# ZcsrenlongZ/Deblur4DGS

Hardware: AMD Instinct MI355X
Metric: Gaussians/s fwd+bwd, 288x512, N_exposure=8 (higher is better)
Workload: dtype f32; 1 GPU; cfg2: 300000 Gaussians (300000 dynamic), 6 motion bases, 512x288, N_exposure=8, 3+depth channels, fwd+bwd to all leaves; gaussians=300000, exposure_subsamples=8, parallelism=1 GPU, lazy_sort=off (auto), pre_roll_steps=30

## Files before the change

### deblur4dgs_amd/csrc/common.h

```cpp
#pragma once
#include <hip/hip_runtime.h>
#include <stdint.h>

#include "../../include/d4gs.h"

#define D4GS_WAVE 64
#define D4GS_MAX_K 32
#define D4GS_PROJ_BLOCK 256


#define D4GS_SSIM_WINDOW                                                                                                   \
  {0.00102838008447911, 0.007598758135239185, 0.03600077212843083, 0.10936068950970002, 0.2130055377112537, 0.26601172486179436, \
   0.2130055377112537,  0.10936068950970002,  0.03600077212843083, 0.007598758135239185, 0.00102838008447911}

void d4gs_set_error(const char *fmt, ...);
int d4gs_check_launch(const char *what);


__device__ __forceinline__ void mat3_mul(const float *A, const float *B, float *C) {
#pragma unroll
  for (int i = 0; i < 3; i++)
#pragma unroll
    for (int j = 0; j < 3; j++) C[i * 3 + j] = A[i * 3] * B[j] + A[i * 3 + 1] * B[3 + j] + A[i * 3 + 2] * B[6 + j];
}
__device__ __forceinline__ void mat3_mul_bt(const float *A, const float *B, float *C) {
#pragma unroll
  for (int i = 0; i < 3; i++)
#pragma unroll
    for (int j = 0; j < 3; j++)
      C[i * 3 + j] = A[i * 3] * B[j * 3] + A[i * 3 + 1] * B[j * 3 + 1] + A[i * 3 + 2] * B[j * 3 + 2];
}
__device__ __forceinline__ void mat3_mul_at(const float *A, const float *B, float *C) {
#pragma unroll
  for (int i = 0; i < 3; i++)
#pragma unroll
    for (int j = 0; j < 3; j++) C[i * 3 + j] = A[i] * B[j] + A[3 + i] * B[3 + j] + A[6 + i] * B[6 + j];
}

__device__ __forceinline__ void quat_to_rotmat(float w, float x, float y, float z, float *R) {
  R[0] = 1.f - 2.f * (y * y + z * z);
  R[1] = 2.f * (x * y - w * z);
  R[2] = 2.f * (x * z + w * y);
  R[3] = 2.f * (x * y + w * z);
  R[4] = 1.f - 2.f * (x * x + z * z);
  R[5] = 2.f * (y * z - w * x);
  R[6] = 2.f * (x * z - w * y);
  R[7] = 2.f * (y * z + w * x);
  R[8] = 1.f - 2.f * (x * x + y * y);
}

struct GS6 {
  float x[3], y[3], z[3];
  float inv_na, inv_nb;
  float d;
};
__device__ __forceinline__ void gram_schmidt(const float *r6, GS6 &o) {
  float na = sqrtf(r6[0] * r6[0] + r6[1] * r6[1] + r6[2] * r6[2]);
  o.inv_na = 1.f / fmaxf(na, 1e-12f);
#pragma unroll
  for (int i = 0; i < 3; i++) o.x[i] = r6[i] * o.inv_na;
  o.d = r6[3] * o.x[0] + r6[4] * o.x[1] + r6[5] * o.x[2];
  float bp[3];
#pragma unroll
  for (int i = 0; i < 3; i++) bp[i] = r6[3 + i] - o.d * o.x[i];
  float nb = sqrtf(bp[0] * bp[0] + bp[1] * bp[1] + bp[2] * bp[2]);
  o.inv_nb = 1.f / fmaxf(nb, 1e-12f);
#pragma unroll
  for (int i = 0; i < 3; i++) o.y[i] = bp[i] * o.inv_nb;
  o.z[0] = o.x[1] * o.y[2] - o.x[2] * o.y[1];
  o.z[1] = o.x[2] * o.y[0] - o.x[0] * o.y[2];
  o.z[2] = o.x[0] * o.y[1] - o.x[1] * o.y[0];
}

__device__ __forceinline__ int rq_choice(const float *R) {
  const float tr = R[0] + R[4] + R[8];
  int ch = 0;
  float best = R[0];
  if (R[4] > best) best = R[4], ch = 1;
  if (R[8] > best) best = R[8], ch = 2;
  if (tr > best) ch = 3;
  return ch;
}
template <int I>
__device__ __forceinline__ void rq_cand(const float *R, float *c) {
  const float tr = R[0] + R[4] + R[8];
  if constexpr (I == 3) {
    c[0] = R[7] - R[5], c[1] = R[2] - R[6], c[2] = R[3] - R[1], c[3] = 1.f + tr;
  } else {
    constexpr int J = (I + 1) % 3, Kk = (I + 2) % 3;
    c[I] = 1.f - tr + 2.f * R[I * 3 + I];
    c[J] = R[J * 3 + I] + R[I * 3 + J];
    c[Kk] = R[Kk * 3 + I] + R[I * 3 + Kk];
    c[3] = R[Kk * 3 + J] - R[J * 3 + Kk];
  }
}
template <int I>
__device__ __forceinline__ void rq_cand_adj(const float *vc, float *vR) {
  if constexpr (I == 3) {
    vR[7] += vc[0], vR[5] -= vc[0], vR[2] += vc[1], vR[6] -= vc[1], vR[3] += vc[2], vR[1] -= vc[2];
    vR[0] += vc[3], vR[4] += vc[3], vR[8] += vc[3];
  } else {
    constexpr int J = (I + 1) % 3, Kk = (I + 2) % 3;
    vR[I * 3 + I] += vc[I], vR[J * 3 + J] -= vc[I], vR[Kk * 3 + Kk] -= vc[I];
    vR[J * 3 + I] += vc[J], vR[I * 3 + J] += vc[J];
    vR[Kk * 3 + I] += vc[Kk], vR[I * 3 + Kk] += vc[Kk];
    vR[Kk * 3 + J] += vc[3], vR[J * 3 + Kk] -= vc[3];
  }
}
__device__ __forceinline__ void rq_cand_dyn(int ch, const float *R, float *c) {
  if (ch == 0) rq_cand<0>(R, c);
  else if (ch == 1) rq_cand<1>(R, c);
  else if (ch == 2) rq_cand<2>(R, c);
  else rq_cand<3>(R, c);
}
__device__ __forceinline__ void rq_cand_adj_dyn(int ch, const float *vc, float *vR) {
  if (ch == 0) rq_cand_adj<0>(vc, vR);
  else if (ch == 1) rq_cand_adj<1>(vc, vR);
  else if (ch == 2) rq_cand_adj<2>(vc, vR);
  else rq_cand_adj<3>(vc, vR);
}
__device__ __forceinline__ void quat_mul(const float *p, const float *q, float *r) {
  r[0] = p[0] * q[0] - p[1] * q[1] - p[2] * q[2] - p[3] * q[3];
  r[1] = p[0] * q[1] + p[1] * q[0] + p[2] * q[3] - p[3] * q[2];
  r[2] = p[0] * q[2] - p[1] * q[3] + p[2] * q[0] + p[3] * q[1];
  r[3] = p[0] * q[3] + p[1] * q[2] - p[2] * q[1] + p[3] * q[0];
}
__device__ __forceinline__ void quat_mul_adj(const float *p, const float *q, const float *vr, float *vp, float *vq) {
  vp[0] = vr[0] * q[0] + vr[1] * q[1] + vr[2] * q[2] + vr[3] * q[3];
  vp[1] = -vr[0] * q[1] + vr[1] * q[0] - vr[2] * q[3] + vr[3] * q[2];
  vp[2] = -vr[0] * q[2] + vr[1] * q[3] + vr[2] * q[0] - vr[3] * q[1];
  vp[3] = -vr[0] * q[3] - vr[1] * q[2] + vr[2] * q[1] + vr[3] * q[0];
  vq[0] = vr[0] * p[0] + vr[1] * p[1] + vr[2] * p[2] + vr[3] * p[3];
  vq[1] = -vr[0] * p[1] + vr[1] * p[0] + vr[2] * p[3] - vr[3] * p[2];
  vq[2] = -vr[0] * p[2] - vr[1] * p[3] + vr[2] * p[0] + vr[3] * p[1];
  vq[3] = -vr[0] * p[3] + vr[1] * p[2] - vr[2] * p[1] + vr[3] * p[0];
}
struct PoseQ {
  int ch;
  float p[4];
  float inv_nc;
  float out[4];
  float inv_nr;
};
__device__ __forceinline__ void pose_quat(const float *Rd, const float *qh, PoseQ &o) {
  float c[4];
  o.ch = rq_choice(Rd);
  rq_cand_dyn(o.ch, Rd, c);
  o.inv_nc = 1.f / sqrtf(c[0] * c[0] + c[1] * c[1] + c[2] * c[2] + c[3] * c[3]);
  o.p[0] = c[3] * o.inv_nc, o.p[1] = c[0] * o.inv_nc, o.p[2] = c[1] * o.inv_nc, o.p[3] = c[2] * o.inv_nc;
  float r[4];
  quat_mul(o.p, qh, r);
  o.inv_nr = 1.f / fmaxf(sqrtf(r[0] * r[0] + r[1] * r[1] + r[2] * r[2] + r[3] * r[3]), 1e-12f);
#pragma unroll
  for (int i = 0; i < 4; i++) o.out[i] = r[i] * o.inv_nr;
}
__device__ __forceinline__ void pose_quat_adj(const PoseQ &o, const float *qh, const float *v_out, float *vRd, float *v_qh) {
  const float dt = v_out[0] * o.out[0] + v_out[1] * o.out[1] + v_out[2] * o.out[2] + v_out[3] * o.out[3];
  float vr[4], vp[4], vq[4];
#pragma unroll
  for (int i = 0; i < 4; i++) vr[i] = (v_out[i] - dt * o.out[i]) * o.inv_nr;
  quat_mul_adj(o.p, qh, vr, vp, vq);
#pragma unroll
  for (int i = 0; i < 4; i++) v_qh[i] += vq[i];
  const float dp = vp[0] * o.p[0] + vp[1] * o.p[1] + vp[2] * o.p[2] + vp[3] * o.p[3];
  float vc[4];
  vc[0] = (vp[1] - dp * o.p[1]) * o.inv_nc, vc[1] = (vp[2] - dp * o.p[2]) * o.inv_nc;
  vc[2] = (vp[3] - dp * o.p[3]) * o.inv_nc, vc[3] = (vp[0] - dp * o.p[0]) * o.inv_nc;
  rq_cand_adj_dyn(o.ch, vc, vRd);
}

__device__ __forceinline__ void tile_rect(float mx, float my, int radius, int tw, int th, int &x0, int &y0, int &x1,
                                          int &y1) {
  const float inv = 1.0f / D4GS_TILE;
  float tx = mx * inv, ty = my * inv, tr = (float)radius * inv;
  x0 = (int)fminf(fmaxf(floorf(tx - tr), 0.f), (float)tw);
  y0 = (int)fminf(fmaxf(floorf(ty - tr), 0.f), (float)th);
  x1 = (int)fminf(fmaxf(ceilf(tx + tr), 0.f), (float)tw);
  y1 = (int)fminf(fmaxf(ceilf(ty + tr), 0.f), (float)th);
}

__device__ __forceinline__ void tight_rect(float mx, float my, float opac, float cov_xx, float cov_yy, int &x0, int &y0,
                                           int &x1, int &y1) {
  const float tau = __logf(255.f * opac) * 1.01f + 0.02f;
  if (!(tau > 0.f)) {
    x1 = x0, y1 = y0;
    return;
  }
  const float ex = sqrtf(2.f * tau * cov_xx) + 1e-3f, ey = sqrtf(2.f * tau * cov_yy) + 1e-3f;
  const float inv = 1.0f / D4GS_TILE;
  const float jx0 = ceilf(mx - ex - 0.5f), jx1 = floorf(mx + ex - 0.5f);
  const float jy0 = ceilf(my - ey - 0.5f), jy1 = floorf(my + ey - 0.5f);
  const int tx0 = (int)fmaxf(floorf(jx0 * inv), (float)x0), tx1 = (int)fminf(floorf(jx1 * inv) + 1.f, (float)x1);
  const int ty0 = (int)fmaxf(floorf(jy0 * inv), (float)y0), ty1 = (int)fminf(floorf(jy1 * inv) + 1.f, (float)y1);
  x0 = tx0, x1 = max(tx1, tx0), y0 = ty0, y1 = max(ty1, ty0);
  if (x1 == x0 || y1 == y0) x1 = x0, y1 = y0;
}

__device__ __forceinline__ bool d4gs_ellipse_hits_rect(float mx, float my, float a, float b, float c, float tau, float X0, float X1,
                                                       float Y0, float Y1) {
  const float U0 = X0 - mx, U1 = X1 - mx, V0 = Y0 - my, V1 = Y1 - my;
  const float uc = fminf(fmaxf(0.f, U0), U1), vc = fminf(fmaxf(0.f, V0), V1);
  if (uc == 0.f && vc == 0.f) return true;
  float best = 3.0e38f;
  if (uc != 0.f) {
    const float v = fminf(fmaxf(-b * uc * __builtin_amdgcn_rcpf(c), V0), V1);
    best = 0.5f * (a * uc * uc + c * v * v) + b * uc * v;
  }
  if (vc != 0.f) {
    const float u = fminf(fmaxf(-b * vc * __builtin_amdgcn_rcpf(a), U0), U1);
    best = fminf(best, 0.5f * (a * u * u + c * vc * vc) + b * u * vc);
  }
  return best <= tau * 1.001f + 1e-4f;
}

struct Cam {
  float R[9];
  float t[3];
  float fx, fy, cx, cy;
  float limx, limy;
};

__device__ __forceinline__ Cam load_cam(const float *V, const float *Km, int width, int height) {
  Cam c;
#pragma unroll
  for (int i = 0; i < 3; i++) {
#pragma unroll
    for (int j = 0; j < 3; j++) c.R[i * 3 + j] = V[i * 4 + j];
    c.t[i] = V[i * 4 + 3];
  }
  c.fx = Km[0], c.fy = Km[4], c.cx = Km[2], c.cy = Km[5];
  c.limx = 1.3f * (0.5f * (float)width / c.fx);
  c.limy = 1.3f * (0.5f * (float)height / c.fy);
  return c;
}

struct ProjOut {
  float pc[3];
  float M[9];
  float covc[6];
  float J02, J12;
  float rz;
  float a, b, c;
  float det;
  float det0;
  float mx, my;
  int radius;
  bool in_x, in_y;
};

__device__ __forceinline__ void project_instance(const Cam &cam, const float *mw, const float *Rm, const float *sc,
                                                 const D4gsDims &d, ProjOut &o) {
  o.radius = 0;
#pragma unroll
  for (int i = 0; i < 3; i++) o.pc[i] = cam.R[i * 3] * mw[0] + cam.R[i * 3 + 1] * mw[1] + cam.R[i * 3 + 2] * mw[2] + cam.t[i];
  float z = o.pc[2];
  if (!(z >= d.near_plane && z <= d.far_plane)) return;
  float W_[9];
  mat3_mul(cam.R, Rm, W_);
#pragma unroll
  for (int i = 0; i < 3; i++)
#pragma unroll
    for (int j = 0; j < 3; j++) o.M[i * 3 + j] = W_[i * 3 + j] * sc[j];
  const float *M = o.M;
  o.covc[0] = M[0] * M[0] + M[1] * M[1] + M[2] * M[2];
  o.covc[1] = M[0] * M[3] + M[1] * M[4] + M[2] * M[5];
  o.covc[2] = M[0] * M[6] + M[1] * M[7] + M[2] * M[8];
  o.covc[3] = M[3] * M[3] + M[4] * M[4] + M[5] * M[5];
  o.covc[4] = M[3] * M[6] + M[4] * M[7] + M[5] * M[8];
  o.covc[5] = M[6] * M[6] + M[7] * M[7] + M[8] * M[8];
  float rz = 1.f / z, rz2 = rz * rz;
  o.rz = rz;
  float xr = o.pc[0] * rz, yr = o.pc[1] * rz;
  o.in_x = (xr <= cam.limx) && (xr >= -cam.limx);
  o.in_y = (yr <= cam.limy) && (yr >= -cam.limy);
  float tx = z * fminf(cam.limx, fmaxf(-cam.limx, xr));
  float ty = z * fminf(cam.limy, fmaxf(-cam.limy, yr));
  float J00 = cam.fx * rz, J11 = cam.fy * rz;
  o.J02 = -cam.fx * tx * rz2;
  o.J12 = -cam.fy * ty * rz2;
  const float cxx = o.covc[0], cxy = o.covc[1], cxz = o.covc[2], cyy = o.covc[3], cyz = o.covc[4], czz = o.covc[5];
  float c00 = J00 * J00 * cxx + 2.f * J00 * o.J02 * cxz + o.J02 * o.J02 * czz;
  float c01 = J00 * J11 * cxy + J00 * o.J12 * cxz + o.J02 * J11 * cyz + o.J02 * o.J12 * czz;
  float c11 = J11 * J11 * cyy + 2.f * J11 * o.J12 * cyz + o.J12 * o.J12 * czz;
  o.a = c00 + d.eps2d;
  o.b = c01;
  o.c = c11 + d.eps2d;
  o.det = o.a * o.c - o.b * o.b;
  o.det0 = __builtin_fmaf(-c01, c01, c00 * c11);
  if (!(o.det > 0.f)) return;
  float mid = 0.5f * (o.a + o.c);
  float v1 = mid + sqrtf(fmaxf(0.01f, mid * mid - o.det));
  float radius = ceilf(3.f * sqrtf(v1));
  if (radius <= d.radius_clip) return;
  o.mx = cam.fx * o.pc[0] * rz + cam.cx;
  o.my = cam.fy * o.pc[1] * rz + cam.cy;
  if (o.mx + radius <= 0.f || o.mx - radius >= (float)d.width || o.my + radius <= 0.f ||
      o.my - radius >= (float)d.height)
    return;
  o.radius = (int)radius;
}

#ifndef D4GS_SEG_MAX
#define D4GS_SEG_MAX 8
#endif
#ifndef D4GS_SEG_UNIT
#define D4GS_SEG_UNIT 256
#endif
#ifndef D4GS_SEG_TILES_MAX
#define D4GS_SEG_TILES_MAX 1280
#endif
#ifndef D4GS_SEG_TILES_MAX_NARROW
#define D4GS_SEG_TILES_MAX_NARROW 5120
#endif
__host__ __device__ __forceinline__ int d4gs_seg_len(int len) {
  const int per = (len + D4GS_SEG_UNIT * D4GS_SEG_MAX - 1) / (D4GS_SEG_UNIT * D4GS_SEG_MAX);
  return D4GS_SEG_UNIT * (per > 1 ? per : 1);
}
int64_t d4gs_seg_state_elems(const D4gsDims *d);
bool d4gs_seg_on(const D4gsDims *d, const D4gsIsect *isect, const D4gsRaster *r);

struct LazyWs {
  int32_t *hist, *near, *pivot, *cur, *flag;
  uint32_t *zr;
  int nb;
};
__host__ __device__ __forceinline__ int d4gs_lazy_buckets(int tiles_per_subsample) { return tiles_per_subsample <= 2048 ? 8 : 4; }
__host__ __device__ __forceinline__ int64_t d4gs_lazy_ws_elems(int S, int tiles_per_subsample) {
  const int64_t T = (int64_t)S * tiles_per_subsample;
  return T * (d4gs_lazy_buckets(tiles_per_subsample) + 5) + 2 * (int64_t)S + 8;
}
__host__ __device__ __forceinline__ LazyWs d4gs_lazy_carve(int32_t *ws, int S, int tiles_per_subsample) {
  LazyWs w;
  const int64_t T = (int64_t)S * tiles_per_subsample;
  w.nb = d4gs_lazy_buckets(tiles_per_subsample);
  w.hist = ws, w.near = w.hist + T * w.nb, w.pivot = w.near + T, w.cur = w.pivot + T, w.flag = w.cur + 2 * T;
  w.zr = reinterpret_cast<uint32_t *>(w.flag + T);
  return w;
}
__device__ __forceinline__ int d4gs_depth_bucket(float depth, uint32_t zmin_bits, uint32_t zmax_bits, int nb) {
  const uint32_t b = __float_as_uint(depth);
  const uint64_t span = (uint64_t)(zmax_bits - zmin_bits) + 1u;
  const uint64_t off = b > zmin_bits ? (uint64_t)(b - zmin_bits) : 0u;
  const int k = (int)((off * (uint64_t)nb) / span);
  return k < nb ? k : nb - 1;
}

struct BlendAdj {
  const float *v_blended;
  const float *v_acc;
  const int8_t *win;
  uint64_t non_mean;
};
bool d4gs_lazy_on(const D4gsDims *d, const D4gsProjOut *out);
int d4gs_lazy_pivot_launch(const D4gsDims *d, const D4gsProjOut *out, int64_t near_target, hipStream_t stream);
int d4gs_lazy_far_sort(const D4gsDims *dims, const D4gsProjOut *proj, const D4gsIsect *isect, hipStream_t stream);
int d4gs_bases_table_launch(const D4gsDims *dims, const D4gsProjIn *in, float *btab, hipStream_t stream);
int d4gs_chunk_per_thread(const D4gsDims *d);
int d4gs_fused_scan_chunks(const D4gsDims *d);

struct ProfScope {
  int slot;
  hipStream_t stream;
  ProfScope(const char *name, hipStream_t s);
  ~ProfScope();
};

__device__ __forceinline__ float splat_sigma2(const float4 g1, float dx, float dy) {
#pragma clang fp contract(off)
  const float inner = __builtin_fmaf(g1.x, dx, g1.y * dy);
  return __builtin_fmaf(dx, inner, (g1.z * dy) * dy);
}
__device__ __forceinline__ float4 stage_conic(float a, float b, float c, float w) {
  constexpr float LOG2E_ = 1.4426950408889634f;
  return make_float4(a * (0.5f * LOG2E_), b * LOG2E_, c * (0.5f * LOG2E_), w);
}

#define D4GS_C1 "quad_perm:[1,0,3,2] row_mask:0xf bank_mask:0xf bound_ctrl:0"
#define D4GS_C2 "quad_perm:[2,3,0,1] row_mask:0xf bank_mask:0xf bound_ctrl:0"
#define D4GS_C3 "row_half_mirror row_mask:0xf bank_mask:0xf bound_ctrl:0"
#define D4GS_C4 "row_mirror row_mask:0xf bank_mask:0xf bound_ctrl:0"
#define D4GS_C5 "row_bcast:15 row_mask:0xa bank_mask:0xf"
#define D4GS_C6 "row_bcast:31 row_mask:0xc bank_mask:0xf"
#define D4GS_DA(i, c) "v_add_f32_dpp %" #i ", %" #i ", %" #i " " c "\n\t"
#define D4GS_S2(c) D4GS_DA(0, c) D4GS_DA(1, c) "s_nop 0\n\t"
#define D4GS_S1(c) D4GS_DA(0, c) "s_nop 1\n\t"

__device__ __forceinline__ float swap32_add(float a, float b) {
  auto r = __builtin_amdgcn_permlane32_swap(__float_as_uint(a), __float_as_uint(b), false, false);
  return __uint_as_float(r[0]) + __uint_as_float(r[1]);
}
__device__ __forceinline__ float swap16_add(float a, float b) {
  auto r = __builtin_amdgcn_permlane16_swap(__float_as_uint(a), __float_as_uint(b), false, false);
  return __uint_as_float(r[0]) + __uint_as_float(r[1]);
}
#define D4GS_R3(c) D4GS_DA(0, c) D4GS_DA(1, c) D4GS_DA(2, c)
__device__ __forceinline__ void rowsum3(float &a, float &b, float &c) {
  asm volatile("s_nop 1\n\t" D4GS_R3(D4GS_C1) D4GS_R3(D4GS_C2) D4GS_R3(D4GS_C3) D4GS_R3(D4GS_C4)
               : "+v"(a), "+v"(b), "+v"(c));
}
__device__ __forceinline__ void rowsum2(float &a, float &b) {
  asm volatile("s_nop 1\n\t" D4GS_S2(D4GS_C1) D4GS_S2(D4GS_C2) D4GS_S2(D4GS_C3) D4GS_S2(D4GS_C4) : "+v"(a), "+v"(b));
}
__device__ __forceinline__ void rowsum1(float &a) {
  asm volatile("s_nop 1\n\t" D4GS_S1(D4GS_C1) D4GS_S1(D4GS_C2) D4GS_S1(D4GS_C3) D4GS_S1(D4GS_C4) : "+v"(a));
}
__device__ __forceinline__ void bcast15(float &a) {
  asm volatile("s_nop 1\n\t" D4GS_DA(0, D4GS_C5) : "+v"(a));
}
__device__ __forceinline__ void bcast15_31(float &a) {
  asm volatile("s_nop 1\n\t" D4GS_DA(0, D4GS_C5) "s_nop 1\n\t" D4GS_DA(0, D4GS_C6) : "+v"(a));
}
template <int NR>
__device__ __forceinline__ void rowsum_all(float (&z)[NR]) {
  constexpr int n3 = NR / 3, r = NR % 3;
#pragma unroll
  for (int i = 0; i < n3; i++) rowsum3(z[3 * i], z[3 * i + 1], z[3 * i + 2]);
  if constexpr (r == 2) rowsum2(z[NR - 2], z[NR - 1]);
  if constexpr (r == 1) rowsum1(z[NR - 1]);
}
#ifndef D4GS_PACKED_LADDER
#define D4GS_PACKED_LADDER 1
#endif
#define D4GS_C7 "row_ror:4 row_mask:0xf bank_mask:0xf"
#define D4GS_C8 "row_ror:8 row_mask:0xf bank_mask:0xf"
#define D4GS_C5S "row_bcast:15 row_mask:0xa bank_mask:0x8"
#define D4GS_C6S "row_bcast:31 row_mask:0xc bank_mask:0x8"
template <bool SINGLE >
__device__ __forceinline__ float rowsum3_packed(float a, float b, float c) {
  const uint64_t odd = 0xaaaaaaaaaaaaaaaaull, l3 = 0x8888888888888888ull;
  if constexpr (SINGLE)
    asm volatile("s_nop 1\n\t" D4GS_R3(D4GS_C1) "v_cndmask_b32_e64 %0, %0, %1, %3\n\ts_nop 0\n\t" D4GS_DA(2, D4GS_C2) D4GS_DA(0, D4GS_C2)
                 "v_cndmask_b32_e64 %0, %0, %2, %4\n\ts_nop 1\n\t" D4GS_DA(0, D4GS_C7) "s_nop 1\n\t" D4GS_DA(0, D4GS_C8)
                 "s_nop 1\n\t" D4GS_DA(0, D4GS_C5S) "s_nop 1\n\t" D4GS_DA(0, D4GS_C6S)
                 : "+v"(a), "+v"(b), "+v"(c)
                 : "s"(odd), "s"(l3));
  else
    asm volatile("s_nop 1\n\t" D4GS_R3(D4GS_C1) "v_cndmask_b32_e64 %0, %0, %1, %3\n\ts_nop 0\n\t" D4GS_DA(2, D4GS_C2) D4GS_DA(0, D4GS_C2)
                 "v_cndmask_b32_e64 %0, %0, %2, %4\n\ts_nop 1\n\t" D4GS_DA(0, D4GS_C7) "s_nop 1\n\t" D4GS_DA(0, D4GS_C8)
                 "s_nop 1\n\t" D4GS_DA(0, D4GS_C5S)
                 : "+v"(a), "+v"(b), "+v"(c)
                 : "s"(odd), "s"(l3));
  return a;
}
template <bool PAIR>
__device__ __forceinline__ float rowsum2_packed(float a, float b) {
  const uint64_t odd = 0xaaaaaaaaaaaaaaaaull;
  if constexpr (PAIR)
    asm volatile("s_nop 1\n\t" D4GS_DA(0, D4GS_C1) D4GS_DA(1, D4GS_C1) "v_cndmask_b32_e64 %0, %0, %1, %2\n\ts_nop 1\n\t" D4GS_DA(0, D4GS_C2)
                 "s_nop 1\n\t" D4GS_DA(0, D4GS_C7) "s_nop 1\n\t" D4GS_DA(0, D4GS_C8) "s_nop 1\n\t" D4GS_DA(0, D4GS_C5S)
                 : "+v"(a), "+v"(b)
                 : "s"(odd));
  else
    asm volatile("s_nop 1\n\t" D4GS_DA(0, D4GS_C1) D4GS_DA(1, D4GS_C1) "v_cndmask_b32_e64 %0, %0, %1, %2\n\ts_nop 1\n\t" D4GS_DA(0, D4GS_C2)
                 "s_nop 1\n\t" D4GS_DA(0, D4GS_C7) "s_nop 1\n\t" D4GS_DA(0, D4GS_C8)
                 : "+v"(a), "+v"(b)
                 : "s"(odd));
  return a;
}
template <int R>
constexpr bool d4gs_wave_sum_split_last() { return D4GS_PACKED_LADDER && R == 7; }
template <int R>
__device__ __forceinline__ void wave_sum_store(float (&v)[R], float *arr, int at, int lane) {
  constexpr int n4 = R / 4, rem = R % 4, n2 = rem / 2, n1 = rem % 2, NR = n4 + n2 + n1;
  if constexpr (D4GS_PACKED_LADDER && n4 == 1 && n2 == 1) {
    const float z0 = swap16_add(swap32_add(v[0], v[1]), swap32_add(v[2], v[3]));
    const float t = swap32_add(v[4], v[5]);
    const int r = lane >> 4, k = lane & 15;
    const int o4 = ((r & 1) << 1) | (r >> 1);
    int ats = at;
    asm volatile("" : "+s"(ats));
    if constexpr (n1) {
      const float q = rowsum2_packed<false>(z0, swap16_add(t, v[6]));
      if (k < 2) arr[ats + (k == 0 ? o4 : (r == 0 ? 4 : r == 1 ? 6 : r == 2 ? 5 : 7))] = q;
    } else {
      const float q = rowsum2_packed<true>(z0, t);
      if (k == 0 || (k == 15 && (r & 1))) arr[ats + (k == 0 ? o4 : 4 + (r >> 1))] = q;
    }
    return;
  }
  float z[NR];
#pragma unroll
  for (int g = 0; g < n4; g++)
    z[g] = swap16_add(swap32_add(v[4 * g], v[4 * g + 1]), swap32_add(v[4 * g + 2], v[4 * g + 3]));
  if constexpr (n2) z[n4] = swap32_add(v[4 * n4], v[4 * n4 + 1]);
  if constexpr (n1) z[NR - 1] = v[R - 1];
  if constexpr (D4GS_PACKED_LADDER && n4 == 2 && n2 + n1 == 1) {
    const float q = rowsum3_packed<n1 == 1>(z[0], z[1], z[2]);
    const int r = lane >> 4, k = lane & 15;
    const int o4 = ((r & 1) << 1) | (r >> 1);
    const bool w = k < 2 || (k == 15 && (n1 ? r == 3 : (r & 1)));
    const int off = k < 2 ? 4 * k + o4 : 8 + (n1 ? 0 : (r >> 1));
    int ats = at;
    asm volatile("" : "+s"(ats));
    if (w) arr[ats + off] = q;
    return;
  }
  rowsum_all(z);
  if constexpr (n2) bcast15(z[n4]);
  if constexpr (n1) bcast15_31(z[NR - 1]);
  if ((lane & 15) == 0) {
    const int r = lane >> 4;
    const int o4 = ((r & 1) << 1) | (r >> 1);
#pragma unroll
    for (int g = 0; g < n4; g++) arr[at + 4 * g + o4] = z[g];
    if constexpr (n2) arr[at + ((r & 1) ? 4 * n4 + (r >> 1) : R)] = z[n4];
    if constexpr (n1) arr[at + (r == 3 ? R - 1 : R)] = z[NR - 1];
  }
}
template <int R>
__device__ __forceinline__ void wave_sum_store(float (&v)[R], float *dst, int lane) {
  wave_sum_store(v, dst, 0, lane);
}

__device__ __forceinline__ uint2 d4gs_pack_box(float x0, float x1, float y0, float y1) {
  const float lo = -32.f, hi = 48.f;
  x0 = fminf(fmaxf(x0 - 0.04f, lo), hi), x1 = fminf(fmaxf(x1 + 0.04f, lo), hi);
  y0 = fminf(fmaxf(y0 - 0.04f, lo), hi), y1 = fminf(fmaxf(y1 + 0.04f, lo), hi);
  typedef _Float16 h2 __attribute__((ext_vector_type(2)));
  const h2 a = {(_Float16)x0, (_Float16)x1}, b = {(_Float16)y0, (_Float16)y1};
  return make_uint2(__builtin_bit_cast(uint32_t, a), __builtin_bit_cast(uint32_t, b));
}
__device__ __forceinline__ float4 d4gs_unpack_box(uint2 p) {
  typedef _Float16 h2 __attribute__((ext_vector_type(2)));
  const h2 a = __builtin_bit_cast(h2, p.x), b = __builtin_bit_cast(h2, p.y);
  return make_float4((float)a[0], (float)a[1], (float)b[0], (float)b[1]);
}


inline int d4gs_lds_pad_for_wgs_per_cu(const void *kernel, int q) {
  if (q <= 0 || q >= 8) return 0;
  hipFuncAttributes at;
  if (hipFuncGetAttributes(&at, kernel) != hipSuccess) return 0;
  const int lds_cu = 160 * 1024, granule = 1280;
  const int need = ((lds_cu / (q + 1) + 1 + granule - 1) / granule) * granule;
  if ((long)need * q > lds_cu) return 0;
  const int pad = need - (int)at.sharedSizeBytes;
  return pad > 0 ? pad : 0;
}

#define D4GS_LAUNCH(name, kernel, grid, block, lds, stream, ...)            \
  do {                                                                        \
    ProfScope _ps(name, stream);                                              \
    hipLaunchKernelGGL(kernel, grid, block, lds, stream, __VA_ARGS__);        \
  } while (0)
```

### deblur4dgs_amd/csrc/raster_fwd.hip

```cpp
#include <stdlib.h>

#include "common.h"

namespace {

struct RasterFwdArgs {
  int N, S, width, height, tw, th;
  int ed;
  const float *geom;
  const float *ctab;
  const float *background;
  const int32_t *tile_offsets;
  const int32_t *sorted_gid;
  float *out;
  float *alphas;
  int32_t *last_ids;
  float *final_T;
  int64_t *n_dev;
  int64_t cap, max_hint;
  float *seg_state;
  const int32_t *lazy_near;
  int32_t *lazy_flag;
  int lazy_pass;
#ifdef D4GS_TRACE
  unsigned long long *trace;
#endif
};
#ifdef D4GS_TRACE
#define D4GS_TCLK(v_) const unsigned long long v_ = wall_clock64();
#define D4GS_TADD(acc_, a_, b_) acc_ += (b_) - (a_);
#else
#define D4GS_TCLK(v_)
#define D4GS_TADD(acc_, a_, b_)
#endif

__device__ __forceinline__ int xcd_remap(int b, int n_blocks) {
  const int per = (n_blocks + 7) >> 3;
  return (b & 7) * per + (b >> 3);
}

#ifdef D4GS_VARIANTS
#include "variants/raster_fwd_variants.inc"
#endif

template <bool PACKED> struct BoxT;
template <> struct BoxT<true> {
  typedef uint2 type;
  static __device__ __forceinline__ uint2 pack(float x0, float x1, float y0, float y1) { return d4gs_pack_box(x0, x1, y0, y1); }
  static __device__ __forceinline__ float4 unpack(uint2 p) { return d4gs_unpack_box(p); }
};
template <> struct BoxT<false> {
  typedef float4 type;
  static __device__ __forceinline__ float4 pack(float x0, float x1, float y0, float y1) { return make_float4(x0, x1, y0, y1); }
  static __device__ __forceinline__ float4 unpack(float4 p) { return p; }
};

template <int B>
__device__ __forceinline__ int d4gs_byte_x16(uint32_t w) {
  int r;
  if constexpr (B == 0) asm("v_lshlrev_b32_sdwa %0, %1, %2 dst_sel:DWORD dst_unused:UNUSED_PAD src0_sel:DWORD src1_sel:BYTE_0" : "=v"(r) : "v"(4u), "v"(w));
  if constexpr (B == 1) asm("v_lshlrev_b32_sdwa %0, %1, %2 dst_sel:DWORD dst_unused:UNUSED_PAD src0_sel:DWORD src1_sel:BYTE_1" : "=v"(r) : "v"(4u), "v"(w));
  if constexpr (B == 2) asm("v_lshlrev_b32_sdwa %0, %1, %2 dst_sel:DWORD dst_unused:UNUSED_PAD src0_sel:DWORD src1_sel:BYTE_2" : "=v"(r) : "v"(4u), "v"(w));
  if constexpr (B == 3) asm("v_lshlrev_b32_sdwa %0, %1, %2 dst_sel:DWORD dst_unused:UNUSED_PAD src0_sel:DWORD src1_sel:BYTE_3" : "=v"(r) : "v"(4u), "v"(w));
  return r;
}
typedef float f32x4_t __attribute__((ext_vector_type(4)));
template <int D, bool DEPTH, bool SEG = false>
__device__ __forceinline__ void raster_fwd_r_body(const RasterFwdArgs &a) {
#pragma clang fp contract(off)
  constexpr int NCH = D + (DEPTH ? 1 : 0);
  constexpr int DP = (D + 3) & ~3;
  constexpr int DV = DP / 4;
  constexpr int FB = (DV > 2 || (SEG && D4GS_SEG_UNIT < 256)) ? 128 : 256;
#ifndef D4GS_FWD_MFMA
#define D4GS_FWD_MFMA 1
#endif
  constexpr bool MF = D4GS_FWD_MFMA && D == 16;
#ifndef D4GS_FWD_NULL0
#define D4GS_FWD_NULL0 1
#endif
#ifndef D4GS_FWD_WIDE4
#define D4GS_FWD_WIDE4 1
#endif
  constexpr bool LIKE_NARROW = DV <= 1 || (MF && D4GS_FWD_WIDE4);
  constexpr bool NULL0 = D4GS_FWD_NULL0 && LIKE_NARROW && !SEG;
  constexpr int FBE = NULL0 ? FB - 1 : FB;
  __shared__ float4 sg0[FB];
  __shared__ float4 sg1[FB];
  __shared__ typename BoxT<(DV <= 1)>::type sbox[FB];
  __shared__ float4 scol[FB * (DV > 0 ? DV : 1)];
  __shared__ __attribute__((aligned(16))) unsigned char slist[4 * 4 * FB];

  D4GS_TCLK(_t0)
#ifdef D4GS_TRACE
  unsigned long long _ts = 0, _tl = 0, _tc = 0, _ti = 0;
  const unsigned long long _c0 = __builtin_amdgcn_s_memtime();
#endif
  if (a.n_dev && (a.n_dev[0] > a.cap || (a.max_hint > 0 && a.n_dev[1] > a.max_hint))) return;
  const int n_tiles_s = a.tw * a.th;
  const int n_tiles = a.S * n_tiles_s;
  const int t = xcd_remap(blockIdx.x, n_tiles);
  if (t >= n_tiles) return;
  const int s = t / n_tiles_s, tl = t - s * n_tiles_s;
  const int ty = tl / a.tw, tx = tl - ty * a.tw;
  const int tid = threadIdx.x, lane = tid & 63, wv = tid >> 6;
  const int row = lane >> 4, kq = lane & 15;
  const int qx0 = tx * D4GS_TILE + (wv & 1) * 8, qy0 = ty * D4GS_TILE + (wv >> 1) * 8;
  const int x = qx0 + (row & 1) * 4 + (kq & 3), y = qy0 + (row >> 1) * 4 + (kq >> 2);
  const bool inside = x < a.width && y < a.height;
  const float pxf = (float)x + 0.5f, pyf = (float)y + 0.5f;
  constexpr bool PB = DV <= 1;
  const float tx0f = PB ? (float)(tx * D4GS_TILE) : 0.f, ty0f = PB ? (float)(ty * D4GS_TILE) : 0.f;
  const float qlx = (float)qx0 - tx0f, qly = (float)qy0 - ty0f;
  const float xl0 = qlx + 0.5f, xh0 = qlx + 3.5f, xl1 = qlx + 4.5f, xh1 = qlx + 7.5f;
  const float yl0 = qly + 0.5f, yh0 = qly + 3.5f, yl1 = qly + 4.5f, yh1 = qly + 7.5f;
  unsigned char *wlist = slist + wv * 4 * FB;
  const unsigned char *mylist = wlist + row * FB;

  float T = 1.f, acc[MF ? (NCH - 16 > 0 ? NCH - 16 : 1) : NCH];
  f32x4_t accm[MF ? 4 : 1];
  int last = 0;
  bool done = !inside, has_last = false;
#pragma unroll
  for (int c = 0; c < (MF ? NCH - 16 : NCH); c++) acc[c] = 0.f;
#pragma unroll
  for (int m = 0; m < (MF ? 4 : 1); m++) accm[m] = f32x4_t{0.f, 0.f, 0.f, 0.f};
  auto chan = [&](int c) -> float {
    if constexpr (MF) return c < 16 ? accm[c & 3][c >> 2] : acc[c - 16];
    else return acc[c];
  };

  const int start = a.tile_offsets[t];
  int end = a.tile_offsets[t + 1];
  const int end_full = end;
  bool has_far = false;
  if (a.lazy_pass == 1) {
    const int nn = a.lazy_near[t];
    has_far = nn < end - start;
    if (has_far && a.lazy_flag[t]) return;
    end = min(end, start + nn);
  } else if (a.lazy_pass == 2 && !a.lazy_flag[t]) return;
  const size_t inst_base = (size_t)s * a.N;
  const int seglen = SEG ? d4gs_seg_len(end_full - start) : 0;
  float *seg_px = SEG ? a.seg_state + (size_t)t * D4GS_SEG_MAX * (1 + NCH) * 256 + ((y - ty * D4GS_TILE) * D4GS_TILE + (x - tx * D4GS_TILE)) : nullptr;
  auto seg_store = [&](int k) {
    if (inside) {
      float *p = seg_px + (size_t)k * (1 + NCH) * 256;
      p[0] = T;
#pragma unroll
      for (int c = 0; c < NCH; c++) p[(1 + c) * 256] = chan(c);
    }
  };
  for (int b = start; b < end; b += FBE) {
    if (__syncthreads_and(done)) break;
    D4GS_TCLK(_ta)
    const int idx = b + tid - (NULL0 ? 1 : 0);
    if (NULL0 && tid == 0) {
      sg0[0] = make_float4(0.f, 0.f, 0.f, 0.f);
      sg1[0] = make_float4(0.f, 0.f, 0.f, 0.f);
      sbox[0] = BoxT<PB>::pack(1e30f, -1e30f, 1e30f, -1e30f);
#pragma unroll
      for (int v = 0; v < DV; v++) scol[v] = make_float4(0.f, 0.f, 0.f, 0.f);
    } else if (tid < FB && idx < end) {
      const int gid = a.sorted_gid[idx];
      const float4 *gp = reinterpret_cast<const float4 *>(a.geom + (inst_base + gid) * D4GS_GEOM_STRIDE);
      const float4 q0 = gp[0], q1 = gp[1];
      sg0[tid] = q0;
      sg1[tid] = stage_conic(q1.x, q1.y, q1.z, 0.f);
      const float tau = __logf(255.f * q0.z) * 1.01f + 0.02f;
      const float det = q1.x * q1.z - q1.y * q1.y;
      const float idet = 1.f / det;
      float ex = -1.f, ey = -1.f;
      if (tau > 0.f && det > 0.f) {
        ex = sqrtf(2.f * tau * q1.z * idet) + 1e-3f;
        ey = sqrtf(2.f * tau * q1.x * idet) + 1e-3f;
      }
      sbox[tid] = ex < 0.f ? BoxT<PB>::pack(1e30f, -1e30f, 1e30f, -1e30f) : BoxT<PB>::pack(q0.x - ex - tx0f, q0.x + ex - tx0f, q0.y - ey - ty0f, q0.y + ey - ty0f);
      const float4 *cp = reinterpret_cast<const float4 *>(a.ctab + (size_t)gid * DP);
#pragma unroll
      for (int v = 0; v < DV; v++) scol[tid * DV + v] = cp[v];
    }
    __syncthreads();
    D4GS_TCLK(_tb)
    D4GS_TADD(_ts, _ta, _tb)
    const int nb = min(FBE, end - b) + (NULL0 ? 1 : 0);
    int c0 = 0, c1 = 0, c2 = 0, c3 = 0;
    constexpr bool NARROW = LIKE_NARROW;
    if constexpr (NARROW) {
      if (lane * 16 < 4 * FB) reinterpret_cast<uint4 *>(wlist)[lane] = make_uint4(0u, 0u, 0u, 0u);
      __builtin_amdgcn_wave_barrier();
    }
#pragma unroll
    for (int k = 0; k < FB / 64; k++) {
      const int jj = k * 64 + lane;
      bool h0 = false, h1 = false, h2 = false, h3 = false;
      if (jj < nb) {
        const float4 bx = BoxT<PB>::unpack(sbox[jj]);
        const bool X0 = (bx.x <= xh0) && (bx.y >= xl0), X1 = (bx.x <= xh1) && (bx.y >= xl1);
        const bool Y0 = (bx.z <= yh0) && (bx.w >= yl0), Y1 = (bx.z <= yh1) && (bx.w >= yl1);
        h0 = X0 && Y0, h1 = X1 && Y0, h2 = X0 && Y1, h3 = X1 && Y1;
      }
      const unsigned long long m0 = __ballot(h0), m1 = __ballot(h1), m2 = __ballot(h2), m3 = __ballot(h3);
      const unsigned char jb = (unsigned char)jj;
      if (h0) wlist[0 * FB + c0 + __builtin_amdgcn_mbcnt_hi((unsigned)(m0 >> 32), __builtin_amdgcn_mbcnt_lo((unsigned)m0, 0u))] = jb;
      if (h1) wlist[1 * FB + c1 + __builtin_amdgcn_mbcnt_hi((unsigned)(m1 >> 32), __builtin_amdgcn_mbcnt_lo((unsigned)m1, 0u))] = jb;
      if (h2) wlist[2 * FB + c2 + __builtin_amdgcn_mbcnt_hi((unsigned)(m2 >> 32), __builtin_amdgcn_mbcnt_lo((unsigned)m2, 0u))] = jb;
      if (h3) wlist[3 * FB + c3 + __builtin_amdgcn_mbcnt_hi((unsigned)(m3 >> 32), __builtin_amdgcn_mbcnt_lo((unsigned)m3, 0u))] = jb;
      c0 += __popcll(m0), c1 += __popcll(m1), c2 += __popcll(m2), c3 += __popcll(m3);
    }
    __builtin_amdgcn_wave_barrier();
    D4GS_TCLK(_tc0)
    D4GS_TADD(_tl, _tb, _tc0)
    const int cnt = row == 0 ? c0 : row == 1 ? c1 : row == 2 ? c2 : c3;
    const int imax = max(max(c0, c1), max(c2, c3));
    int last16 = -1;
    unsigned long long donem = __builtin_amdgcn_ballot_w64(done);
    auto step = [&](const unsigned long long actm, const int j16 ) {
      const float4 g0 = *reinterpret_cast<const float4 *>(reinterpret_cast<const char *>(sg0) + j16);
      const float4 g1 = *reinterpret_cast<const float4 *>(reinterpret_cast<const char *>(sg1) + j16);
      const float dx = g0.x - pxf, dy = g0.y - pyf;
      const float sigma = splat_sigma2(g1, dx, dy);
      const float alpha = fminf(0.999f, g0.z * __builtin_amdgcn_exp2f(-sigma));
      const float nT = T * (1.f - alpha);
      const unsigned long long vm = (NULL0 ? ~0ull : actm) & __builtin_amdgcn_ballot_w64(sigma >= 0.f) & __builtin_amdgcn_ballot_w64(alpha >= (1.f / 255.f)) & ~donem;
      const unsigned long long mm = __builtin_amdgcn_ballot_w64(nT > 1e-4f);
      donem |= vm & ~mm;
      const bool valid = __builtin_amdgcn_inverse_ballot_w64(vm & mm);
      const float vis = valid ? alpha * T : 0.f;
      if constexpr (MF) {
        const float4 ct = *reinterpret_cast<const float4 *>(reinterpret_cast<const char *>(scol) + j16 * DV + 16 * (lane & 3));
        accm[0] = __builtin_amdgcn_mfma_f32_4x4x1f32(ct.x, vis, accm[0], 0, 0, 0);
        accm[1] = __builtin_amdgcn_mfma_f32_4x4x1f32(ct.y, vis, accm[1], 0, 0, 0);
        accm[2] = __builtin_amdgcn_mfma_f32_4x4x1f32(ct.z, vis, accm[2], 0, 0, 0);
        accm[3] = __builtin_amdgcn_mfma_f32_4x4x1f32(ct.w, vis, accm[3], 0, 0, 0);
        if (DEPTH) acc[0] = __builtin_fmaf(g0.w, vis, acc[0]);
      } else {
#pragma unroll
        for (int v = 0; v < DV; v++) {
          const float4 c4 = *reinterpret_cast<const float4 *>(reinterpret_cast<const char *>(scol) + j16 * DV + 16 * v);
          if (v * 4 < D) acc[v * 4] = __builtin_fmaf(c4.x, vis, acc[v * 4]);
          if (v * 4 + 1 < D) acc[v * 4 + 1] = __builtin_fmaf(c4.y, vis, acc[v * 4 + 1]);
          if (v * 4 + 2 < D) acc[v * 4 + 2] = __builtin_fmaf(c4.z, vis, acc[v * 4 + 2]);
          if (v * 4 + 3 < D) acc[v * 4 + 3] = __builtin_fmaf(c4.w, vis, acc[v * 4 + 3]);
        }
        if (DEPTH) acc[D] = __builtin_fmaf(g0.w, vis, acc[D]);
      }
      T = valid ? nT : T;
      last16 = valid ? j16 : last16;
    };
#ifndef D4GS_FWD_LIST4
#define D4GS_FWD_LIST4 1
#endif
    if constexpr (D4GS_FWD_LIST4 && NARROW) {
      for (int i0 = 0; i0 < imax; i0 += 16) {
        const int i1 = min(i0 + 16, imax);
        for (int i = i0; i < i1; i += 4) {
          const uint32_t w4 = *reinterpret_cast<const uint32_t *>(mylist + i);
          step(NULL0 ? 0ull : __builtin_amdgcn_ballot_w64(i < cnt), d4gs_byte_x16<0>(w4));
          step(NULL0 ? 0ull : __builtin_amdgcn_ballot_w64(i + 1 < cnt), d4gs_byte_x16<1>(w4));
          step(NULL0 ? 0ull : __builtin_amdgcn_ballot_w64(i + 2 < cnt), d4gs_byte_x16<2>(w4));
          step(NULL0 ? 0ull : __builtin_amdgcn_ballot_w64(i + 3 < cnt), d4gs_byte_x16<3>(w4));
        }
        if (donem == ~0ull) break;
      }
      done = __builtin_amdgcn_inverse_ballot_w64(donem);
    } else {
      for (int i0 = 0; i0 < imax; i0 += 16) {
        const int i1 = min(i0 + 16, imax);
        for (int i = i0; i < i1; i++) {
          const bool act = i < cnt;
          const int jr = (int)mylist[i];
          const int j = act ? jr : 0;
          const float4 g0 = sg0[j], g1 = sg1[j];
          const float dx = g0.x - pxf, dy = g0.y - pyf;
          const float sigma = splat_sigma2(g1, dx, dy);
          const float alpha = fminf(0.999f, g0.z * __builtin_amdgcn_exp2f(-sigma));
          bool valid = act && !done && (sigma >= 0.f) && (alpha >= (1.f / 255.f));
          const float nT = T * (1.f - alpha);
          const bool sat = nT <= 1e-4f;
          done = done || (valid && sat);
          valid = valid && !sat;
          const float vis = valid ? alpha * T : 0.f;
          if constexpr (MF) {
            const float4 ct = scol[j * 4 + (lane & 3)];
            accm[0] = __builtin_amdgcn_mfma_f32_4x4x1f32(ct.x, vis, accm[0], 0, 0, 0);
            accm[1] = __builtin_amdgcn_mfma_f32_4x4x1f32(ct.y, vis, accm[1], 0, 0, 0);
            accm[2] = __builtin_amdgcn_mfma_f32_4x4x1f32(ct.z, vis, accm[2], 0, 0, 0);
            accm[3] = __builtin_amdgcn_mfma_f32_4x4x1f32(ct.w, vis, accm[3], 0, 0, 0);
            if (DEPTH) acc[0] = __builtin_fmaf(g0.w, vis, acc[0]);
          } else {
#pragma unroll
            for (int v = 0; v < DV; v++) {
              const float4 c4 = scol[j * DV + v];
              if (v * 4 < D) acc[v * 4] = __builtin_fmaf(c4.x, vis, acc[v * 4]);
              if (v * 4 + 1 < D) acc[v * 4 + 1] = __builtin_fmaf(c4.y, vis, acc[v * 4 + 1]);
              if (v * 4 + 2 < D) acc[v * 4 + 2] = __builtin_fmaf(c4.z, vis, acc[v * 4 + 2]);
              if (v * 4 + 3 < D) acc[v * 4 + 3] = __builtin_fmaf(c4.w, vis, acc[v * 4 + 3]);
            }
            if (DEPTH) acc[D] = __builtin_fmaf(g0.w, vis, acc[D]);
          }
          T = valid ? nT : T;
          last16 = valid ? 16 * j : last16;
        }
        if (__all(done)) break;
      }
    }
    last = last16 >= 0 ? b + (last16 >> 4) - (NULL0 ? 1 : 0) : last;
    has_last = has_last || last16 >= 0;
    D4GS_TCLK(_tc1)
    D4GS_TADD(_tc, _tc0, _tc1)
#ifdef D4GS_TRACE
    _ti += (unsigned long long)imax;
#endif
    if constexpr (SEG) {
      const int e = b + FB - start;
      if (e < end - start && e % seglen == 0) seg_store(e / seglen);
    }
  }
  if (has_far) {
    if (!__syncthreads_and(done)) {
      if (tid == 0) a.lazy_flag[t] = 1;
      return;
    }
  }
  if (a.lazy_pass == 2 && tid == 0) a.lazy_flag[t] = 2;
  if constexpr (SEG) seg_store(0);

  const int lstride = (n_tiles + 127) >> 7;
  if (a.n_dev && t % lstride == 0) {
    __shared__ int slive_hi[4];
    int hi = (inside && last >= start && has_last) ? last : start - 1;
#pragma unroll
    for (int o = 32; o > 0; o >>= 1) hi = max(hi, __shfl_xor(hi, o));
    if (lane == 0) slive_hi[wv] = hi;
    __syncthreads();
    if (tid == 0) {
      const int h = max(max(slive_hi[0], slive_hi[1]), max(slive_hi[2], slive_hi[3]));
      atomicAdd(reinterpret_cast<unsigned long long *>(a.n_dev + 2), (unsigned long long)(end_full - start));
      atomicAdd(reinterpret_cast<unsigned long long *>(a.n_dev + 3), (unsigned long long)(h - start + 1));
    }
  }
  if (inside) {
    const size_t pix = ((size_t)s * a.height + y) * a.width + x;
    const float al = 1.f - T;
    a.alphas[pix] = al;
    a.final_T[pix] = T;
    a.last_ids[pix] = last;
    float *o = a.out + pix * NCH;
#pragma unroll
    for (int c = 0; c < D; c++) o[c] = chan(c) + (a.background ? T * a.background[c] : 0.f);
    if (DEPTH) o[D] = a.ed ? chan(D) / fmaxf(al, 1e-10f) : chan(D);
  }
#ifdef D4GS_TRACE
  if (a.trace && tid == 0) {
    unsigned long long *tr = a.trace + (size_t)blockIdx.x * 10;
    tr[8] = __builtin_amdgcn_s_memtime() - _c0;
    tr[0] = _t0, tr[1] = wall_clock64(), tr[3] = (unsigned long long)(end - start), tr[4] = _ts, tr[5] = _tl, tr[6] = _tc, tr[7] = _ti;
    tr[2] = __builtin_amdgcn_s_getreg((4 << 0) | (0 << 6) | (31 << 11)) | ((unsigned long long)__builtin_amdgcn_s_getreg((20 << 0) | (0 << 6) | (31 << 11)) << 32);
  }
#endif
}
template <int D, bool DEPTH>
__global__ void __launch_bounds__(256) __attribute__((amdgpu_waves_per_eu(8, 8))) k_raster_fwd_r8(const RasterFwdArgs a) {
  raster_fwd_r_body<D, DEPTH>(a);
}
#ifndef D4GS_FWD_WIDE_WAVES
#define D4GS_FWD_WIDE_WAVES 6
#endif
template <int D, bool DEPTH>
__global__ void __launch_bounds__(256)
#if D4GS_FWD_WIDE_WAVES > 0
__attribute__((amdgpu_waves_per_eu(D == 16 ? D4GS_FWD_WIDE_WAVES : 1, D == 16 ? D4GS_FWD_WIDE_WAVES : 10)))
#endif
k_raster_fwd_r(const RasterFwdArgs a) {
  raster_fwd_r_body<D, DEPTH>(a);
}
template <int D, bool DEPTH>
__global__ void __launch_bounds__(256) __attribute__((amdgpu_waves_per_eu(8, 8))) k_raster_fwd_rs8(const RasterFwdArgs a) {
  raster_fwd_r_body<D, DEPTH, true>(a);
}
template <int D, bool DEPTH>
__global__ void __launch_bounds__(256)
#if D4GS_FWD_WIDE_WAVES > 0
__attribute__((amdgpu_waves_per_eu(D == 16 ? D4GS_FWD_WIDE_WAVES : 1, D == 16 ? D4GS_FWD_WIDE_WAVES : 10)))
#endif
k_raster_fwd_rs(const RasterFwdArgs a) {
  raster_fwd_r_body<D, DEPTH, true>(a);
}

template <int D, bool DEPTH>
int launch_fwd(const RasterFwdArgs &a, hipStream_t stream) {
  const int n_tiles = a.S * a.tw * a.th;
  const int blocks = ((n_tiles + 7) / 8) * 8;
#ifdef D4GS_VARIANTS
  static const bool wave_per_tile = getenv("D4GS_FWD_WAVE_PER_TILE") != nullptr;
  static const bool quads = getenv("D4GS_FWD_QUADS") != nullptr;
  if constexpr (D > 0) {
    if (wave_per_tile) {
      D4GS_LAUNCH("k_raster_fwd", (k_raster_fwd<D, DEPTH>), dim3(blocks), dim3(64), 0, stream, a);
      return d4gs_check_launch("k_raster_fwd");
    }
    if (quads) {
      D4GS_LAUNCH("k_raster_fwd_q", (k_raster_fwd_q<D, DEPTH>), dim3(blocks), dim3(256), 0, stream, a);
      return d4gs_check_launch("k_raster_fwd_q");
    }
  }
#endif
  if (a.seg_state) {
    if constexpr (D <= 4) D4GS_LAUNCH("k_raster_fwd_r", (k_raster_fwd_rs8<D, DEPTH>), dim3(blocks), dim3(256), 0, stream, a);
    else D4GS_LAUNCH("k_raster_fwd_r", (k_raster_fwd_rs<D, DEPTH>), dim3(blocks), dim3(256), 0, stream, a);
    return d4gs_check_launch("k_raster_fwd_r");
  }
  static const int q_env = getenv("D4GS_FWD_Q") ? atoi(getenv("D4GS_FWD_Q")) : 0;
  if constexpr (D <= 4) {
    const int pad = d4gs_lds_pad_for_wgs_per_cu((const void *)k_raster_fwd_r8<D, DEPTH>, q_env);
    D4GS_LAUNCH("k_raster_fwd_r", (k_raster_fwd_r8<D, DEPTH>), dim3(blocks), dim3(256), pad, stream, a);
  } else {
    const int pad = d4gs_lds_pad_for_wgs_per_cu((const void *)k_raster_fwd_r<D, DEPTH>, q_env);
    D4GS_LAUNCH("k_raster_fwd_r", (k_raster_fwd_r<D, DEPTH>), dim3(blocks), dim3(256), pad, stream, a);
  }
  return d4gs_check_launch("k_raster_fwd_r");
}

}

int64_t d4gs_seg_state_elems(const D4gsDims *d) {
  const int64_t tw = (d->width + D4GS_TILE - 1) / D4GS_TILE, th = (d->height + D4GS_TILE - 1) / D4GS_TILE;
  const int64_t n_tiles = (int64_t)d->S * tw * th;
  if (n_tiles > (d->D <= 4 ? D4GS_SEG_TILES_MAX_NARROW : D4GS_SEG_TILES_MAX)) return 0;
  const int64_t nch = d->D + (d->depth_mode != D4GS_DEPTH_NONE ? 1 : 0);
  return n_tiles * D4GS_SEG_MAX * (1 + nch) * 256;
}
bool d4gs_seg_on(const D4gsDims *d, const D4gsIsect *isect, const D4gsRaster *r) {
  const char *env = getenv("D4GS_SEG");
  if (!r->seg_state || d4gs_seg_state_elems(d) == 0 || (env && env[0] == '0')) return false;
#ifdef D4GS_VARIANTS
  if (getenv("D4GS_FWD_WAVE_PER_TILE") || getenv("D4GS_FWD_QUADS") || getenv("D4GS_BWD_WAVE_PER_TILE") || getenv("D4GS_BWD_MFMA"))
    return false;
#endif
  if (env && env[0] == '1') return true;
  return isect->max_tile_count > D4GS_SEG_UNIT;
}

int d4gs_raster_fwd_impl(const D4gsDims *dims, const D4gsProjOut *proj, const D4gsIsect *isect, const D4gsRaster *r,
                         hipStream_t stream) {
  RasterFwdArgs a;
  a.N = dims->N, a.S = dims->S, a.width = dims->width, a.height = dims->height;
  a.tw = (dims->width + D4GS_TILE - 1) / D4GS_TILE;
  a.th = (dims->height + D4GS_TILE - 1) / D4GS_TILE;
  a.ed = dims->depth_mode == D4GS_DEPTH_ED;
  a.geom = proj->geom, a.ctab = proj->ctab, a.background = r->background;
  a.tile_offsets = proj->tile_offsets, a.sorted_gid = isect->sorted_gid;
  a.n_dev = proj->n_isect, a.cap = isect->n_isect, a.max_hint = isect->max_tile_count;
  a.out = r->render_colors, a.alphas = r->render_alphas, a.last_ids = r->last_ids, a.final_T = r->final_T;
  a.seg_state = d4gs_seg_on(dims, isect, r) ? r->seg_state : nullptr;
  a.lazy_near = nullptr, a.lazy_flag = nullptr, a.lazy_pass = 0;
  const bool lazy = d4gs_lazy_on(dims, proj) && isect->n_isect > 0;
  if (lazy) {
    const LazyWs lw = d4gs_lazy_carve(proj->lazy_ws, dims->S, a.tw * a.th);
    a.lazy_near = lw.near, a.lazy_flag = lw.flag, a.lazy_pass = 1;
  }
#ifdef D4GS_TRACE
  a.trace = getenv("D4GS_TRACE_FWD_PTR") ? (unsigned long long *)strtoull(getenv("D4GS_TRACE_FWD_PTR"), nullptr, 0) : nullptr;
#endif
  const bool dep = dims->depth_mode != D4GS_DEPTH_NONE;
  auto launch = [&](const RasterFwdArgs &aa) -> int {
#define D4GS_CASE(DD)                                                   \
  case DD:                                                              \
    return dep ? launch_fwd<DD, true>(aa, stream) : launch_fwd<DD, false>(aa, stream);
    switch (dims->D) {
      case 0:
        if (dep) return launch_fwd<0, true>(aa, stream);
        d4gs_set_error("D = 0 needs a depth mode (the depth-only composite)");
        return D4GS_EINVAL;
      D4GS_CASE(1)
      D4GS_CASE(2)
      D4GS_CASE(3)
      D4GS_CASE(4)
      D4GS_CASE(5)
      D4GS_CASE(8)
      D4GS_CASE(16)
      default:
        d4gs_set_error("unsupported colour channel count D=%d (instantiated: 1,2,3,4,5,8,16; render wider colour "
                       "vectors in chunks over the same projection / tile lists)", dims->D);
        return D4GS_EINVAL;
    }
#undef D4GS_CASE
  };
  int rc = launch(a);
  if (rc || !lazy) return rc;
  if ((rc = d4gs_lazy_far_sort(dims, proj, isect, stream))) return rc;
  a.lazy_pass = 2;
  return launch(a);
}
```

Measured before the change: 250.1 million Gaussians/s.

## Add exact per-block conic culling of staged Gaussians before forward compositing

After the bounding-box ballot builds per-row candidate lists, each 16-lane group now finds the minimum of the conic quadratic over its 4x4 pixel block. It drops Gaussians whose minimum exceeds the alpha threshold (tau stored in the conic's w slot), then compacts the list and recomputes imax. Waves whose pixels are all saturated skip list building entirely. This removes wasted per-pixel alpha evaluations for Gaussians whose box overlaps the block but whose ellipse does not reach it, at the cost of an extra filtering pass over each list. The filter is on by default, can be disabled through an environment variable, and a test kernel for it is added.

Result: faster. 253.3 million Gaussians/s, median of 6 (+1.3%).

```diff
diff --git a/deblur4dgs_amd/csrc/common.h b/deblur4dgs_amd/csrc/common.h
--- a/deblur4dgs_amd/csrc/common.h
+++ b/deblur4dgs_amd/csrc/common.h
@@ -375,6 +375,17 @@
   return make_float4(a * (0.5f * LOG2E_), b * LOG2E_, c * (0.5f * LOG2E_), w);
 }
 
+__device__ __forceinline__ float d4gs_alpha_tau(float opac) { return __logf(255.f * opac) * 1.01f + 0.02f; }
+__device__ __forceinline__ bool d4gs_block_filter_keep(float mx, float my, const float4 g1, float X0, float X1, float Y0, float Y1) {
+#pragma clang fp contract(off)
+  const float U0 = X0 - mx, U1 = X1 - mx, V0 = Y0 - my, V1 = Y1 - my;
+  const float uc = __builtin_amdgcn_fmed3f(0.f, U0, U1), vc = __builtin_amdgcn_fmed3f(0.f, V0, V1);
+  const float v = __builtin_amdgcn_fmed3f((g1.y * uc) * __builtin_amdgcn_rcpf(-2.f * g1.z), V0, V1);
+  const float u = __builtin_amdgcn_fmed3f((g1.y * vc) * __builtin_amdgcn_rcpf(-2.f * g1.x), U0, U1);
+  const float best = fminf(splat_sigma2(g1, uc, v), splat_sigma2(g1, u, vc));
+  return !(best > g1.w * 1.001f + 1.5e-4f);
+}
+
 #define D4GS_C1 "quad_perm:[1,0,3,2] row_mask:0xf bank_mask:0xf bound_ctrl:0"
 #define D4GS_C2 "quad_perm:[2,3,0,1] row_mask:0xf bank_mask:0xf bound_ctrl:0"
 #define D4GS_C3 "row_half_mirror row_mask:0xf bank_mask:0xf bound_ctrl:0"
diff --git a/deblur4dgs_amd/csrc/raster_fwd.hip b/deblur4dgs_amd/csrc/raster_fwd.hip
--- a/deblur4dgs_amd/csrc/raster_fwd.hip
+++ b/deblur4dgs_amd/csrc/raster_fwd.hip
@@ -22,6 +22,7 @@
   const int32_t *lazy_near;
   int32_t *lazy_flag;
   int lazy_pass;
+  int block_filter;
 #ifdef D4GS_TRACE
   unsigned long long *trace;
 #endif
@@ -166,8 +167,8 @@
       const float4 *gp = reinterpret_cast<const float4 *>(a.geom + (inst_base + gid) * D4GS_GEOM_STRIDE);
       const float4 q0 = gp[0], q1 = gp[1];
       sg0[tid] = q0;
-      sg1[tid] = stage_conic(q1.x, q1.y, q1.z, 0.f);
-      const float tau = __logf(255.f * q0.z) * 1.01f + 0.02f;
+      const float tau = d4gs_alpha_tau(q0.z);
+      sg1[tid] = stage_conic(q1.x, q1.y, q1.z, tau * 1.4426950408889634f);
       const float det = q1.x * q1.z - q1.y * q1.y;
       const float idet = 1.f / det;
       float ex = -1.f, ey = -1.f;
@@ -183,7 +184,8 @@
     __syncthreads();
     D4GS_TCLK(_tb)
     D4GS_TADD(_ts, _ta, _tb)
-    const int nb = min(FBE, end - b) + (NULL0 ? 1 : 0);
+    const bool wave_live = __builtin_amdgcn_ballot_w64(done) != ~0ull;
+    const int nb = wave_live ? min(FBE, end - b) + (NULL0 ? 1 : 0) : 0;
     int c0 = 0, c1 = 0, c2 = 0, c3 = 0;
     constexpr bool NARROW = LIKE_NARROW;
     if constexpr (NARROW) {
@@ -209,10 +211,37 @@
       c0 += __popcll(m0), c1 += __popcll(m1), c2 += __popcll(m2), c3 += __popcll(m3);
     }
     __builtin_amdgcn_wave_barrier();
+    int cnt = row == 0 ? c0 : row == 1 ? c1 : row == 2 ? c2 : c3;
+    int imax = max(max(c0, c1), max(c2, c3));
+    if (a.block_filter) {
+      int lf = lane;
+      asm volatile("" : "+v"(lf));
+      const int kf = lf & 15, rsh = lf & 48;
+      unsigned char *mylist_w = wlist + rsh * (FB / 16);
+      const float X0 = pxf - (float)(kf & 3), Y0 = pyf - (float)(kf >> 2);
+      const float X1 = X0 + 3.f, Y1 = Y0 + 3.f;
+      const unsigned below = (1u << kf) - 1u;
+      int n = 0;
+      for (int i = 0; i < imax; i += 16) {
+        const int p = i + kf;
+        bool keep = false;
+        unsigned char jb = 0;
+        if (p < cnt) {
+          jb = mylist_w[p];
+          const float4 g0 = sg0[jb], g1 = sg1[jb];
+          keep = d4gs_block_filter_keep(g0.x, g0.y, g1, X0, X1, Y0, Y1);
+          if constexpr (NULL0) mylist_w[p] = 0;
+        }
+        const unsigned m16 = (unsigned)(__builtin_amdgcn_ballot_w64(keep) >> rsh) & 0xffffu;
+        if (keep) mylist_w[n + __popc(m16 & below)] = jb;
+        n += __popc(m16);
+      }
+      cnt = n;
+      imax = max(max(__builtin_amdgcn_readlane(n, 0), __builtin_amdgcn_readlane(n, 16)), max(__builtin_amdgcn_readlane(n, 32), __builtin_amdgcn_readlane(n, 48)));
+      __builtin_amdgcn_wave_barrier();
+    }
     D4GS_TCLK(_tc0)
     D4GS_TADD(_tl, _tb, _tc0)
-    const int cnt = row == 0 ? c0 : row == 1 ? c1 : row == 2 ? c2 : c3;
-    const int imax = max(max(c0, c1), max(c2, c3));
     int last16 = -1;
     unsigned long long donem = __builtin_amdgcn_ballot_w64(done);
     auto step = [&](const unsigned long long actm, const int j16 ) {
@@ -455,6 +484,8 @@
   a.out = r->render_colors, a.alphas = r->render_alphas, a.last_ids = r->last_ids, a.final_T = r->final_T;
   a.seg_state = d4gs_seg_on(dims, isect, r) ? r->seg_state : nullptr;
   a.lazy_near = nullptr, a.lazy_flag = nullptr, a.lazy_pass = 0;
+  const char *bf = getenv("D4GS_BLOCK_FILTER");
+  a.block_filter = !(bf && bf[0] == '0');
   const bool lazy = d4gs_lazy_on(dims, proj) && isect->n_isect > 0;
   if (lazy) {
     const LazyWs lw = d4gs_lazy_carve(proj->lazy_ws, dims->S, a.tw * a.th);
@@ -493,3 +524,20 @@
   a.lazy_pass = 2;
   return launch(a);
 }
+
+#ifdef D4GS_VARIANTS
+namespace {
+__global__ void __launch_bounds__(64) k_test_block_filter(int n, const float *rec, int32_t *keep) {
+  const int i = blockIdx.x * 64 + threadIdx.x;
+  if (i >= n) return;
+  const float *r = rec + (size_t)i * 10;
+  const float4 g1 = stage_conic(r[3], r[4], r[5], d4gs_alpha_tau(r[2]) * 1.4426950408889634f);
+  keep[i] = d4gs_block_filter_keep(r[0], r[1], g1, r[6], r[7], r[8], r[9]) ? 1 : 0;
+}
+}
+extern "C" D4GS_API int d4gs_test_block_filter(int n, const float *rec, int32_t *keep, void *stream) {
+  if (n <= 0) return D4GS_EINVAL;
+  hipLaunchKernelGGL(k_test_block_filter, dim3((n + 63) / 64), dim3(64), 0, (hipStream_t)stream, n, rec, keep);
+  return hipGetLastError() == hipSuccess ? 0 : D4GS_ELAUNCH;
+}
+#endif
```
